# Raymond30/Krylov-Cubic-Regularized-Newton

Hardware: AMD Instinct MI355X
Metric: Hessian-vector products/sec + achieved HBM GB/s, news20 CSR, 1/2/4/8 MI355X (higher is better)
Workload: dtype f64; 1 GPU; news20: one device Lanczos (cubic.py:77-111) of m=100 HVPs per step; n=19996, d=1355191, nnz=9097916, m=100, partition=none, parallelism=single GPU

## Files before the change

krylov-cubic-regularized-newton_amd/csrc/krcn_geom.hpp:

```cpp
#pragma once
#include <stdint.h>

#include <cstdlib>
#include <cstring>

#include "krcn.h"

#ifdef __HIPCC__
#define KRCN_HD __host__ __device__
#else
#define KRCN_HD
#endif

namespace krcn {

constexpr int kNumCUs = 256;
constexpr int kNT = 256;
constexpr int kMaxPartials = 2048;

constexpr int kApplyU = 4;
inline int apply_grid(int64_t rows) {
  int64_t b = (rows + int64_t(kNT) * kApplyU - 1) / (int64_t(kNT) * kApplyU);
  return int(b < 1 ? 1 : (b > 1024 ? 1024 : b));
}

inline const char* tuning_env(const char* name) {
#ifdef KRCN_TUNING
  return getenv(name);
#else
  (void)name;
  return nullptr;
#endif
}
template <typename V>
inline V tuning_value(const char* name, V dflt, int field = 0) {
  const char* e = tuning_env(name);
  for (; e && field > 0; --field)
    if ((e = std::strchr(e, ',')) != nullptr) ++e;
  return e ? V(std::atof(e)) : dflt;
}
inline bool tuning_on(const char* name) {
  const char* e = tuning_env(name);
  return !(e && e[0] == '0');
}
inline bool tuning_off(const char* name) {
  const char* e = tuning_env(name);
  return e && e[0] == '1';
}

inline int auto_lanes(int64_t rows, int64_t nnz) {
  const double mean = rows > 0 ? double(nnz) / double(rows) : 0.0;
  int L = 1;
  while (L < 64 && double(L * 2) * 8.0 <= mean) L *= 2;
  return L;
}

inline int resolve_lanes(int policy, int64_t rows, int64_t nnz) {
  if (policy == KRCN_LANES_AUTO) return auto_lanes(rows, nnz);
  if (policy == KRCN_LANES_SEQUENTIAL) return 1;
  return policy;
}

struct __attribute__((aligned(32))) TileDesc {
  int slice, long_row, row0, row1, p0, p1, pad0, pad1;
};

constexpr int kWaveTileNnz = 512;
constexpr int kWaveTileRows = 128;
constexpr int kWavesPerBlock = kNT / 64;

constexpr int kCombineRows = 128;
constexpr int kCombineSpread = 256;
inline int combine_rows(int rows) {
  const int R = (rows + kCombineSpread - 1) / kCombineSpread;
  return R < 1 ? 1 : (R > kCombineRows ? kCombineRows : R);
}
inline int combine_grid(int rows) {
  const int R = combine_rows(rows);
  const int g = (rows + R - 1) / R;
  return g < 1 ? 1 : (g > kCombineSpread ? kCombineSpread : g);
}

constexpr int kSortPerThread = 8;
constexpr int ilog2(int v) { return v <= 1 ? 0 : 1 + ilog2(v / 2); }
template <int NT> struct SortGeom {
  static constexpr int kTile = NT * kSortPerThread;
  static constexpr int kRows = kTile / 4;
  static constexpr int kRowRegs = (kRows + 1 + NT - 1) / NT;
  static constexpr int kSlotBits = ilog2(kTile);
  static_assert((1 << kSlotBits) == kTile, "slot field must address a whole tile");
  static constexpr int64_t kMaxWindow = int64_t(1) << (32 - kSlotBits);
};

struct __attribute__((aligned(16))) WinSeg {
  int slice, t0, t1, flags;
};
enum { kSegLoad = 1, kSegFlush = 2 };

constexpr int kWinNT = 1024;
constexpr int kWinWaves = kWinNT / 64;
constexpr int kWinChunk = 256;
constexpr int kWinTMax = 6;
constexpr int kWinPad = kWinChunk + 8;
constexpr int kWinRing = 3;
constexpr int kWinBatch = 26;
template <typename T> struct WinGeom {
  static constexpr int kSlabBytes = kWinWaves * kWinChunk * int(sizeof(T));
  static constexpr int kBytes = 163840 - kSlabBytes - 256;
  static constexpr int kW = kBytes / int(sizeof(T));
  static constexpr int kPer = (kW + kWinNT - 1) / kWinNT;
  static_assert(kW <= 65536, "16-bit slice-local offsets");
};

KRCN_HD inline void win_block_slice(int b, int G, int S, int kpb, int& slice, int& chunk) {
  if (kpb == 0) {
    slice = b % S;
    chunk = b / S;
    return;
  }
  const int x = b % 8, q = G / 8, r = G % 8;
  const int slot = x * q + (x < r ? x : r) + b / 8;
  slice = slot / kpb;
  chunk = slot % kpb;
}

constexpr int kXtChunk = 4;
constexpr int kXtRowCap = kWinWaves * kWinTMax * 64;
constexpr unsigned short kXtPad = 0xFFFF;
template <typename T> struct XtGeom {
  static constexpr int kChunks = WinGeom<T>::kW - kWinNT - kXtRowCap;
};

constexpr int kJagNT = 1024;
constexpr int kJagWaves = kJagNT / 64;
constexpr int kJagLdsBytes = 163840 - 256;
constexpr int kJagPieces = kJagLdsBytes / 16;
constexpr int kJagSlab = 128;
constexpr int kJagPad = 2 * kJagSlab;

#ifndef KRCN_JAG_CPG
#define KRCN_JAG_CPG 2
#endif
constexpr int kJagK1 = 6, kJagCPG1 = KRCN_JAG_CPG, kJagLC = 8;
constexpr int kJagCPGU = 2;
constexpr int jag_cpg(int K) { return K <= 2 ? 2 : kJagCPG1; }
constexpr int kJagK2 = 8;
constexpr int kJagLong = 32, kJagTask = 128, kJagLongTasks = 256;

template <typename T> struct JagGeom {
  static constexpr int kE = 16 / int(sizeof(T));
  static constexpr int kW1 = kJagPieces * kE;
  static constexpr int kR1 = (kJagPieces + kJagNT - 1) / kJagNT;
  static constexpr int kPieces2 = (kJagLdsBytes - kJagWaves * (kJagSlab + 2) * int(sizeof(T))) / 32;
  static constexpr int kW2 = kPieces2 * kE;
  static constexpr int kR2 = (kPieces2 + kJagNT - 1) / kJagNT;
  static_assert(kW1 <= 65536, "16-bit slice-local offsets");
};

}
```

krylov-cubic-regularized-newton_amd/csrc/krcn_window.hpp:

```cpp
#pragma once
#include <type_traits>
#include <utility>

#include "krcn_tiled.hpp"

namespace krcn {

#ifndef KRCN_WIN_RING_ACCUM
#define KRCN_WIN_RING_ACCUM 2
#endif
constexpr int kWinRingAccum = KRCN_WIN_RING_ACCUM;
#ifndef KRCN_WIN_SUMU
#define KRCN_WIN_SUMU 8
#endif
#ifndef KRCN_WIN_COOP
#define KRCN_WIN_COOP 1
#endif
constexpr int kWinCoopLen = 64;
#ifndef KRCN_WIN_FIRST
#define KRCN_WIN_FIRST 1
#endif

struct WinArgs {
  int rows, W, stride, S;
  int dbg;
  int ntiles;
  int64_t cols;
  const int* tb;
  const unsigned short* ro;
  const unsigned short* widx;
  const void* wval;
  const WinSeg* segs;
  int kpb = 0;
};
template <bool kAccum>
__device__ __forceinline__ const int* win_tb(const WinArgs& a, int slice) {
  return a.tb + int64_t(slice) * ((kAccum ? 1 : 2) * (a.ntiles + 1));
}

typedef unsigned short u16x4 __attribute__((ext_vector_type(4)));

template <typename T> struct Quad;
template <> struct Quad<double> {
  __device__ __forceinline__ static void load(const double* p, double (&v)[4]) {
    const f64x2 a = *reinterpret_cast<const f64x2*>(p);
    const f64x2 b = *(reinterpret_cast<const f64x2*>(p) + 1);
    v[0] = a.x; v[1] = a.y; v[2] = b.x; v[3] = b.y;
  }
};
template <> struct Quad<float> {
  __device__ __forceinline__ static void load(const float* p, float (&v)[4]) {
    const f32x4 a = *reinterpret_cast<const f32x4*>(p);
    v[0] = a.x; v[1] = a.y; v[2] = a.z; v[3] = a.w;
  }
};

#ifdef KRCN_WIN_TIMING
constexpr int kWinDbgSlots = 32;
static __device__ unsigned long long krcn_win_dbg[3 * 2048 * kWinDbgSlots];
[[maybe_unused]] static int win_stamps_read(unsigned long long* out, int n, int reset) {
  if (hipDeviceSynchronize() != hipSuccess) return 1;
  if (hipMemcpyFromSymbol(out, HIP_SYMBOL(krcn_win_dbg), sizeof(unsigned long long) * n) != hipSuccess) return 1;
  if (reset) {
    static unsigned long long z[3 * 2048 * kWinDbgSlots];
    if (hipMemcpyToSymbol(HIP_SYMBOL(krcn_win_dbg), z, sizeof(z)) != hipSuccess) return 1;
  }
  return 0;
}
#define KRCN_WIN_STAMP(slot)                                                                          \
  do {                                                                                                \
    if (threadIdx.x == 0 && blockIdx.x < 2048)                                                        \
      krcn_win_dbg[a.dbg * 2048 * kWinDbgSlots + blockIdx.x * kWinDbgSlots + (slot)] =   \
          __builtin_amdgcn_s_memrealtime();                                                           \
  } while (0)
#define KRCN_WIN_WAVE_STAMP(slot)                                                                     \
  do {                                                                                                \
    if ((threadIdx.x & 63) == 0 && blockIdx.x < 2048)                                                 \
      krcn_win_dbg[a.dbg * 2048 * kWinDbgSlots + blockIdx.x * kWinDbgSlots + (slot)] =   \
          __builtin_amdgcn_s_memrealtime();                                                           \
  } while (0)
#else
#define KRCN_WIN_STAMP(slot) do {} while (0)
#define KRCN_WIN_WAVE_STAMP(slot) do {} while (0)
#endif

template <typename T, typename TS = T> struct WinChunk {
  u16x4 q;
  TS v[4];
  int c0, base, hi;
};

template <typename T, typename TS>
__device__ __forceinline__ void win_load(WinChunk<T, TS>& c, int c0, int e1, const unsigned short* __restrict__ widx,
                                         const TS* __restrict__ wval, int lane) {
  c.c0 = c0;
  c.base = c0 & ~3;
  c.hi = c.base + kWinChunk < e1 ? c.base + kWinChunk : e1;
  const int e = c.base + 4 * lane;
  c.q = *reinterpret_cast<const u16x4*>(widx + e);
  Quad<TS>::load(wval + e, c.v);
}

template <typename T, typename TS>
__device__ __forceinline__ T win_consume(const WinChunk<T, TS>& c, int beg, int end, const T* win, T* slab, int lane,
                                         T s, bool coop, T& open) {
  const int e = c.base + 4 * lane;
  const unsigned short qi[4] = {c.q.x, c.q.y, c.q.z, c.q.w};
#if defined(KRCN_WIN_ABL_NOSUM)
#pragma unroll
  for (int i = 0; i < 4; ++i) s += T(c.v[i]) * win[e + i < c.hi ? qi[i] : 0];
  (void)beg; (void)end; (void)slab; (void)coop; (void)open;
  return s;
#else
#pragma unroll
  for (int i = 0; i < 4; ++i) slab[4 * lane + i] = T(c.v[i]) * win[e + i < c.hi ? qi[i] : 0];
  wave_lds_sync();
  const int pb = beg > c.c0 ? beg : c.c0;
  const int pe = end < c.hi ? end : c.hi;
  int p = pb;
#if KRCN_WIN_SUMU > 1
  if (coop) {
    unsigned long long longm = __ballot(end - beg > kWinCoopLen && pe > pb);
    while (longm != 0ull) {
      const int L = __builtin_ctzll(longm);
      longm &= longm - 1ull;
      const int lb = __builtin_amdgcn_readlane(pb, L), le = __builtin_amdgcn_readlane(pe, L);
      const int rb = __builtin_amdgcn_readlane(beg, L), re = __builtin_amdgcn_readlane(end, L);
      T part = lb > rb ? open : T(0);
      for (int q = lb + ((lane - (lb - rb)) & 63); q < le; q += 64) part += slab[q - c.base];
      if (le < re) {
        open = part;
        continue;
      }
#pragma unroll
      for (int off = 32; off > 0; off >>= 1) part += __shfl_xor(part, off, 64);
      if (lane == L) s += part;
    }
    if (end - beg > kWinCoopLen) p = pe;
  }
  if (__ballot(pe - p > 2 * KRCN_WIN_SUMU) != 0ull) {
    for (; p + KRCN_WIN_SUMU <= pe; p += KRCN_WIN_SUMU) {
      T a[KRCN_WIN_SUMU];
#pragma unroll
      for (int u = 0; u < KRCN_WIN_SUMU; ++u) a[u] = slab[p + u - c.base];
#pragma unroll
      for (int u = 0; u < KRCN_WIN_SUMU; ++u) s += a[u];
    }
  }
#endif
  for (; p < pe; ++p) s += slab[p - c.base];
  wave_lds_sync();
  return s;
#endif
}

__device__ __forceinline__ void lds_block_barrier() {
  __builtin_amdgcn_fence(__ATOMIC_RELEASE, "workgroup", "local");
  __builtin_amdgcn_s_barrier();
  __builtin_amdgcn_fence(__ATOMIC_ACQUIRE, "workgroup", "local");
}

template <typename T>
__device__ __forceinline__ void win_fetch(T (&tmp)[WinGeom<T>::kPer], const T* __restrict__ x, int slice,
                                          const WinArgs& a, int rot) {
  constexpr int kPer = WinGeom<T>::kPer;
  const int64_t wbase = int64_t(slice) * a.W;
  const int len = a.cols - wbase < a.W ? int(a.cols - wbase) : a.W;
#pragma unroll
  for (int k = 0; k < kPer; ++k) {
    const int q = k + rot < kPer ? k + rot : k + rot - kPer;
    const int i = threadIdx.x + kWinNT * q;
    if (kWinNT * q < len) tmp[k] = x[wbase + (i < len ? i : len - 1)];
  }
}

template <typename T>
__device__ __forceinline__ void win_store(const T (&tmp)[WinGeom<T>::kPer], T* win, int slice, const WinArgs& a,
                                          int rot) {
  constexpr int kPer = WinGeom<T>::kPer;
  const int64_t wbase = int64_t(slice) * a.W;
  const int len = a.cols - wbase < a.W ? int(a.cols - wbase) : a.W;
#pragma unroll
  for (int k = 0; k < kPer; ++k) {
    const int q = k + rot < kPer ? k + rot : k + rot - kPer;
    const int i = threadIdx.x + kWinNT * q;
    if (i < len) win[i] = tmp[k];
  }
}

template <int... I, class F>
__device__ __forceinline__ void unroll_while(std::integer_sequence<int, I...>, int n, F&& f) {
  bool go = true;
  ((go = go && (I < n), go ? (f(std::integral_constant<int, I>{}), 0) : 0), ...);
}

template <int R>
struct TileB {
  int r0, nr, e0, e1;
  __device__ __forceinline__ void set(int rows, int t, int t1, int te0, int te1) {
    t = t < t1 ? t : t1 - 1;
    t = t > 0 ? t : 0;
    r0 = t * R;
    nr = rows - r0 < R ? rows - r0 : R;
    e0 = te0;
    e1 = te1;
  }
  __device__ __forceinline__ void set_rows(int tr0, int tr1, int te0, int te1) {
    r0 = tr0;
    nr = tr1 - tr0;
    e0 = te0;
    e1 = te1;
  }
};

struct WinTiles {
  int lo, hi, kb;
  template <bool kRows>
  __device__ __forceinline__ void load(const int* tb, int roff, int tw, int t1, int kb_, int lane) {
    kb = kb_;
    int t = tw + kWinWaves * (kb + (kRows ? lane & 31 : lane));
    t = t < t1 ? t : t1 - 1;
    t = t > 0 ? t : 0;
    if (kRows && lane >= 32) t += roff;
    lo = tb[t];
    hi = tb[t + 1];
  }
};

struct RowRaw {
  int o1, o0;
};
template <int R>
__device__ __forceinline__ RowRaw tile_row_load(const TileB<R>& b, const unsigned short* ro, int lane) {
  const int i1 = lane < b.nr ? lane : b.nr - 1;
  const int i0 = lane < b.nr ? (lane > 0 ? lane - 1 : 0) : b.nr - 1;
  return RowRaw{int(ro[b.r0 + i1]), int(ro[b.r0 + i0])};
}
template <int R>
__device__ __forceinline__ void tile_row_bounds(const TileB<R>& b, const RowRaw& q, int lane, int& bg, int& en) {
  const int ea = b.e0 + q.o1, eb = b.e0 + q.o0;
  en = lane < b.nr ? ea : b.e1;
  bg = lane < b.nr ? (lane > 0 ? eb : b.e0) : b.e1;
}

#ifndef KRCN_FOLD
#define KRCN_FOLD 0
#endif
#ifndef KRCN_FOLD_ABL
#define KRCN_FOLD_ABL 0
#endif
constexpr int kFoldPad = 32;
template <typename T> struct EpiSliceFold {
  T* part; int64_t ld;
  int* cnt;
  int* won;
  int* nwon;
  int ntiles;
  double* aq;
  const T* w; T* u;
  LzCtl<T> c;
  int S;
  static constexpr bool kReduce = false;
  struct Pre {};
  template <class Src> __device__ __forceinline__ void init(const Src&) {}
  __device__ __forceinline__ Pre pre(int) const { return Pre{}; }
  __device__ __forceinline__ double row(int r, T s, int slice, const Pre&) const {
    __hip_atomic_store(part + int64_t(slice) * ld + r, s, __ATOMIC_RELAXED, __HIP_MEMORY_SCOPE_AGENT);
    return 0.0;
  }
};
template <class E> struct IsFoldEpi : std::false_type {};
template <typename T> struct IsFoldEpi<EpiSliceFold<T>> : std::true_type {};

template <typename T>
__device__ __forceinline__ double fold_beta(const LzCtl<T>& c, int lane) {
  double g[kNT / 64];
#pragma unroll
  for (int w = 0; w < kNT / 64; ++w) {
    double v = 0.0;
    for (int i = 64 * w + lane; i < c.Pnorm; i += kNT) v += c.pnorm[i];
    g[w] = wave_sum(v);
  }
  return sqrt((g[0] + g[1]) + (g[2] + g[3]));
}

struct WinFold {
  int t1 = -1, t2 = -1;
  int a1 = -1, a2 = -1;
  int o1 = 0, o2 = 0;
  int bstate = 0;
  double beta = 0.0;
};

template <typename T, int R>
__device__ __forceinline__ void fold_combine(const EpiSliceFold<T>& e, WinFold& f, int t, int rows, int lane) {
  if constexpr (R != 32) {
    return;
  } else {
  if (f.bstate == 0) {
    const int done = e.c.j > 0 ? __hip_atomic_load(&e.c.st->done, __ATOMIC_RELAXED, __HIP_MEMORY_SCOPE_AGENT) : 0;
    f.beta = fold_beta(e.c, lane);
    f.bstate = (done || (e.c.j > 0 && fabs(f.beta) < e.c.tol)) ? 2 : 1;
  }
  const int r0 = t * R;
  if (f.bstate == 1) {
    __builtin_amdgcn_fence(__ATOMIC_ACQUIRE, "agent");
    const int p = lane & 15, q = lane >> 4;
    const int ra = r0 + 2 * p;
    const int rA = ra < rows ? ra : rows - 1, rB = ra + 1 < rows ? ra + 1 : rows - 1;
    T w0 = T(0), w1 = T(0);
    if (q == 0) {
      w0 = e.w[rA];
      w1 = e.w[rB];
    }
    constexpr int kH = 12;
    T v0a = T(0), v4a = T(0), v0b = T(0), v4b = T(0);
#pragma unroll
    for (int h = 0; h < 2; ++h) {
      T a0[kH], a1[kH];
#pragma unroll
      for (int k = 0; k < kH; ++k) {
        const int s = q + 4 * (h * kH + k);
        const T* pp = e.part + int64_t(s < e.S ? s : q) * e.ld;
        a0[k] = __hip_atomic_load(pp + rA, __ATOMIC_RELAXED, __HIP_MEMORY_SCOPE_AGENT);
        a1[k] = __hip_atomic_load(pp + rB, __ATOMIC_RELAXED, __HIP_MEMORY_SCOPE_AGENT);
      }
#pragma unroll
      for (int k = 0; k < kH; ++k)
        if (q + 4 * (h * kH + k) < e.S) {
          if (k % 2 == 0) { v0a += a0[k]; v0b += a1[k]; }
          else { v4a += a0[k]; v4b += a1[k]; }
        }
    }
    const T n0a = __shfl_down(v0a, 16, 64), n4a = __shfl_down(v4a, 16, 64);
    const T n0b = __shfl_down(v0b, 16, 64), n4b = __shfl_down(v4b, 16, 64);
    const T l1a = v0a + n0a, l5a = v4a + n4a, l1b = v0b + n0b, l5b = v4b + n4b;
    const T m1a = __shfl_down(l1a, 32, 64), m5a = __shfl_down(l5a, 32, 64);
    const T m1b = __shfl_down(l1b, 32, 64), m5b = __shfl_down(l5b, 32, 64);
    const T sa = (l1a + m1a) + (l5a + m5a), sb = (l1b + m1b) + (l5b + m5b);
    double acc = 0.0;
    if (q == 0) {
      const T div = T(f.beta);
      if (ra < rows) {
        const T qa = sa / div, ua = w0 * qa;
        e.u[ra] = ua;
        acc += double(ua) * double(qa);
      }
      if (ra + 1 < rows) {
        const T qb = sb / div, ub = w1 * qb;
        e.u[ra + 1] = ub;
        acc += double(ub) * double(qb);
      }
    }
    acc = wave_sum(acc);
    if (lane == 0) e.aq[t] = acc;
  } else if (lane == 0) {
    e.aq[t] = 0.0;
  }
  if (lane == 0) __hip_atomic_store(e.cnt + int64_t(t) * kFoldPad, 0, __ATOMIC_RELAXED, __HIP_MEMORY_SCOPE_AGENT);
  }
}

template <typename T>
__device__ __forceinline__ void fold_won(const EpiSliceFold<T>& e, int t, int lane) {
  if (lane == 0) {
    const int i = __hip_atomic_fetch_add(e.nwon, 1, __ATOMIC_RELAXED, __HIP_MEMORY_SCOPE_WORKGROUP);
    e.won[int64_t(blockIdx.x) * e.ntiles + i] = t;
  }
}

template <typename T, int R>
__device__ __forceinline__ void fold_after(const EpiSliceFold<T>& e, WinFold& f, int t, int rows, int lane) {
  if (f.a2 >= 0 && __builtin_amdgcn_readfirstlane(f.o2) == e.S - 1) fold_won(e, f.a2, lane);
  f.a2 = f.a1;
  f.o2 = f.o1;
  f.a1 = -1;
  if (f.t2 >= 0) {
    __builtin_amdgcn_s_waitcnt(0x0f78);
    int o = 0;
#if KRCN_FOLD_ABL
    if (lane == 0) o = f.t2 % 97 == 0 ? 0 : 1;
#else
    if (lane == 0) o = __hip_atomic_fetch_add(e.cnt + int64_t(f.t2) * kFoldPad, 1, __ATOMIC_RELAXED, __HIP_MEMORY_SCOPE_AGENT);
#endif
    f.o1 = o;
    f.a1 = f.t2;
  }
  f.t2 = f.t1;
  f.t1 = t;
}

template <typename T, int R>
__device__ __forceinline__ void fold_drain(const EpiSliceFold<T>& e, WinFold& f, int rows, int lane) {
  __builtin_amdgcn_s_waitcnt(0x0f70);
  int ta[4] = {f.a2, f.a1, f.t2, f.t1};
  int oa[4] = {f.o2, f.o1, 0, 0};
#pragma unroll
  for (int i = 2; i < 4; ++i)
    if (ta[i] >= 0) {
      int o = 0;
      if (lane == 0) o = __hip_atomic_fetch_add(e.cnt + int64_t(ta[i]) * kFoldPad, 1, __ATOMIC_RELAXED, __HIP_MEMORY_SCOPE_AGENT);
      oa[i] = o;
    }
#pragma unroll
  for (int i = 0; i < 4; ++i)
    if (ta[i] >= 0 && __builtin_amdgcn_readfirstlane(oa[i]) == e.S - 1) fold_won(e, ta[i], lane);
  f = WinFold{};
}

template <typename T, typename TS, int R, class Epi>
__device__ __forceinline__ void win_stream(int segno, const WinSeg& sg, const WinArgs& a,
                                           const T (&tmp)[WinGeom<T>::kPer], bool store_win, int rot, T* win,
                                           T* slab, const Epi& epi, int wave, int lane,
                                           typename RedOf<Epi>::type& red, WinTiles tl) {
  const int rows = a.rows;
  const int* tb = win_tb<false>(a, sg.slice);
  const unsigned short* ro = a.ro + int64_t(sg.slice) * rows;
  const unsigned short* widx = a.widx;
  const TS* wval = static_cast<const TS*>(a.wval);
  const int tw = sg.t0 + wave;
  const int nt = sg.t1 - tw > 0 ? (sg.t1 - tw + kWinWaves - 1) / kWinWaves : 0;
  const int nb = (nt + kWinBatch - 1) / kWinBatch;
  WinFold fold;
  if (nb == 0 && store_win) {
    lds_block_barrier();
    win_store<T>(tmp, win, sg.slice, a, rot);
    lds_block_barrier();
  }
  for (int bi = 0; bi < nb; ++bi) {
    const int kb = bi * kWinBatch;
    const int kn = nt - kb < kWinBatch ? nt - kb : kWinBatch;
    if (bi > 0) tl.load<true>(tb, a.ntiles + 1, tw, sg.t1, kb, lane);
    auto bounds = [&](TileB<R>& b, int k) {
      b.e0 = __builtin_amdgcn_readlane(tl.lo, k);
      b.e1 = __builtin_amdgcn_readlane(tl.hi, k);
    };
    TileB<R> B0, B1, B2;
    bounds(B0, 0);
    bounds(B1, 1);
    bounds(B2, 2);
    WinChunk<T, TS> c0, c1, c2;
    RowRaw q0, q1, q2;
    typename Epi::Pre p0, p1, p2;
    auto rows_of = [&](TileB<R>& b, int k, RowRaw& q, typename Epi::Pre& pr) {
      b.set_rows(__builtin_amdgcn_readlane(tl.lo, k + 32), __builtin_amdgcn_readlane(tl.hi, k + 32), b.e0, b.e1);
      q = tile_row_load<R>(b, ro, lane);
      const int r = b.r0 + lane;
      pr = epi.pre(r < rows ? r : rows - 1);
    };
    const bool sw = bi == 0 && store_win;
#if KRCN_WIN_FIRST
    if (sw) {
      lds_block_barrier();
      win_store<T>(tmp, win, sg.slice, a, rot);
    }
    rows_of(B0, 0, q0, p0);
    win_load(c0, B0.e0, B0.e1, widx, wval, lane);
    win_load(c1, B1.e0, B1.e1, widx, wval, lane);
    if (sw) lds_block_barrier();
#else
    rows_of(B0, 0, q0, p0);
    win_load(c0, B0.e0, B0.e1, widx, wval, lane);
    win_load(c1, B1.e0, B1.e1, widx, wval, lane);
    if (sw) {
      lds_block_barrier();
      win_store<T>(tmp, win, sg.slice, a, rot);
      lds_block_barrier();
    }
#endif
    if (segno < 4 && bi == 0) KRCN_WIN_STAMP(2 + 2 * segno);
    auto finish = [&](const WinChunk<T, TS>& c, const TileB<R>& b, const RowRaw& q, const typename Epi::Pre& pr,
                      int k) {
      int bg, en;
      tile_row_bounds<R>(b, q, lane, bg, en);
      const bool coop = KRCN_WIN_COOP && a.S > 1;
      T open = T(0);
      T s = win_consume(c, bg, en, win, slab, lane, T(0), coop, open);
      for (int cc = c.hi; cc < b.e1;) {
        WinChunk<T, TS> cx;
        win_load(cx, cc, b.e1, widx, wval, lane);
        s = win_consume(cx, bg, en, win, slab, lane, s, coop, open);
        cc = cx.hi;
      }
      if (k < kn && lane < b.nr) red += epi.row(b.r0 + lane, s, sg.slice, pr);
      if constexpr (IsFoldEpi<Epi>::value)
        if (k < kn) fold_after<T, R>(epi, fold, b.r0 / R, rows, lane);
    };
    for (int k = 0; k < kn; k += 3) {
      rows_of(B1, k + 1, q1, p1);
      win_load(c2, B2.e0, B2.e1, widx, wval, lane);
      finish(c0, B0, q0, p0, k);
      bounds(B0, k + 3);
      rows_of(B2, k + 2, q2, p2);
      win_load(c0, B0.e0, B0.e1, widx, wval, lane);
      finish(c1, B1, q1, p1, k + 1);
      bounds(B1, k + 4);
      rows_of(B0, k + 3, q0, p0);
      win_load(c1, B1.e0, B1.e1, widx, wval, lane);
      finish(c2, B2, q2, p2, k + 2);
      bounds(B2, k + 5);
    }
  }
  if constexpr (IsFoldEpi<Epi>::value) fold_drain<T, R>(epi, fold, rows, lane);
}

template <typename T, typename TS, int R, class Epi, bool FLUSH>
__device__ __forceinline__ void win_accum(int segno, const WinSeg& sg, const WinArgs& a, const T (&tmp)[WinGeom<T>::kPer],
                                          bool store_win, int rot, T* win, T* slab, const Epi& epi, int wave,
                                          int lane, T (&acc)[kWinTMax], typename RedOf<Epi>::type& red,
                                          const WinTiles& tl) {
  constexpr int K = kWinTMax;
  constexpr int D = kWinRingAccum;
  const int rows = a.rows;
  const unsigned short* ro = a.ro + int64_t(sg.slice) * rows;
  const unsigned short* widx = a.widx;
  const TS* wval = static_cast<const TS*>(a.wval);
  const int nt = sg.t1 - sg.t0 - wave > 0 ? (sg.t1 - sg.t0 - wave + kWinWaves - 1) / kWinWaves : 0;
  TileB<R> B[K];
#pragma unroll
  for (int k = 0; k < K; ++k)
    B[k].set(rows, sg.t0 + wave + k * kWinWaves, sg.t1, __builtin_amdgcn_readlane(tl.lo, k),
             __builtin_amdgcn_readlane(tl.hi, k));
  WinChunk<T, TS> ring[D];
  RowRaw rq[D];
  typename Epi::Pre pre[D];
  auto issue_chunk = [&](auto kc) {
    constexpr int k = decltype(kc)::value;
    win_load(ring[k % D], B[k].e0, B[k].e1, widx, wval, lane);
  };
  auto issue_rows = [&](auto kc) {
    constexpr int k = decltype(kc)::value;
    rq[k % D] = tile_row_load<R>(B[k], ro, lane);
    if constexpr (FLUSH) {
      const int r = B[k].r0 + lane;
      pre[k % D] = epi.pre(r < rows ? r : rows - 1);
    }
  };
#if KRCN_WIN_FIRST
  if (store_win) {
    lds_block_barrier();
    win_store<T>(tmp, win, sg.slice, a, rot);
  }
  issue_rows(std::integral_constant<int, 0>{});
  issue_chunk(std::integral_constant<int, 0>{});
  if constexpr (K > 1 && D > 2) issue_chunk(std::integral_constant<int, 1>{});
  if (store_win) lds_block_barrier();
#else
  issue_rows(std::integral_constant<int, 0>{});
  issue_chunk(std::integral_constant<int, 0>{});
  if constexpr (K > 1 && D > 2) issue_chunk(std::integral_constant<int, 1>{});
  if (store_win) {
    lds_block_barrier();
    win_store<T>(tmp, win, sg.slice, a, rot);
    lds_block_barrier();
  }
#endif
  if (segno < 4) KRCN_WIN_STAMP(2 + 2 * segno);
  auto step = [&](auto kc) {
    constexpr int k = decltype(kc)::value;
    if constexpr (k + 1 < K) issue_rows(std::integral_constant<int, k + 1>{});
    if constexpr (k + D - 1 < K && D > 1) issue_chunk(std::integral_constant<int, k + D - 1>{});
    const WinChunk<T, TS>& cur = ring[k % D];
    int bg, en;
    tile_row_bounds<R>(B[k], rq[k % D], lane, bg, en);
    T none = T(0);
    T s = win_consume(cur, bg, en, win, slab, lane, acc[k], false, none);
    for (int c = cur.hi; c < B[k].e1;) {
      WinChunk<T, TS> cx;
      win_load(cx, c, B[k].e1, widx, wval, lane);
      s = win_consume(cx, bg, en, win, slab, lane, s, false, none);
      c = cx.hi;
    }
    if constexpr (FLUSH) {
      if (lane < B[k].nr) red += epi.row(B[k].r0 + lane, s, sg.slice, pre[k % D]);
      acc[k] = T(0);
    } else {
      acc[k] = s;
    }
  };
  unroll_while(std::make_integer_sequence<int, K>{}, nt, step);
}

template <typename T> struct EpiLz1X {
  const T* w; T div;
  const int* xcp;
  const unsigned short* xrow;
  const T* xval;
  T* part;
  int cols;
  T* lu; int rbase;
  static constexpr bool kReduce = false;
  static constexpr bool kPreEarly = true;
  struct Pre { T wr; };
  template <class S> __device__ __forceinline__ void init(const S& src) { div = src.v.div; }
  __device__ __forceinline__ Pre pre(int r) const { return Pre{w[r]}; }
  __device__ __forceinline__ double row(int r, T s, int, const Pre& p) const {
    lu[r - rbase] = p.wr * (s / div);
    return 0.0;
  }
  __device__ __forceinline__ void xt(int b, T* tp) const {
    const int* cp = xcp + int64_t(b) * (cols + 1);
    const int c = threadIdx.x;
    const int cb = cp[0], ce = cp[cols];
    int c0 = 0, c1 = 0;
    if (c < cols) {
      c0 = cp[c];
      c1 = cp[c + 1];
    }
    for (int t = cb + int(threadIdx.x); t < ce; t += kWinNT) {
      T v[kXtChunk];
      Quad<T>::load(xval + int64_t(t) * kXtChunk, v);
      const u16x4 q = *reinterpret_cast<const u16x4*>(xrow + int64_t(t) * kXtChunk);
      const unsigned short rr[kXtChunk] = {q.x, q.y, q.z, q.w};
      T s = T(0);
#pragma unroll
      for (int i = 0; i < kXtChunk; ++i) {
        const T pr = v[i] * lu[rr[i] != kXtPad ? rr[i] : 0];
        if (rr[i] != kXtPad) s += pr;
      }
      tp[t - cb] = s;
    }
    __builtin_amdgcn_fence(__ATOMIC_RELEASE, "workgroup", "local");
    __builtin_amdgcn_s_barrier();
    __builtin_amdgcn_fence(__ATOMIC_ACQUIRE, "workgroup", "local");
    if (c < cols) {
      T s = T(0);
      for (int k = c0; k < c1; ++k) s += tp[k - cb];
      part[int64_t(b) * cols + c] = s;
    }
  }
};
template <class E> struct IsEpiXt : std::false_type {};
template <typename T> struct IsEpiXt<EpiLz1X<T>> : std::true_type {};


template <typename T, typename TS, int R, class Src, class Epi, bool kAccum>
__global__ __launch_bounds__(kWinNT, 1) void k_window_pass(WinArgs a, Src src, Epi epi,
                                                           double* __restrict__ partials) {
  constexpr int kPer = WinGeom<T>::kPer;
  __shared__ double sm[kWinNT / 64];
  __shared__ T win[WinGeom<T>::kW];
  __shared__ T slab_all[kWinWaves][kWinChunk];
  __shared__ int fold_n;
  if constexpr (IsFoldEpi<Epi>::value) {
    if (threadIdx.x == 0) fold_n = 0;
    epi.nwon = &fold_n;
  }
  KRCN_WIN_STAMP(0);
  const WinSeg* bsegs = a.segs + int64_t(blockIdx.x) * a.stride;
  WinSeg sg = bsegs[0];
  const int nseg = sg.flags >> 8;
  const int rot = int((blockIdx.x >> 3) % kPer);
  int slice0 = sg.slice, chunk0 = 0;
  if constexpr (!kAccum) win_block_slice(int(blockIdx.x), int(gridDim.x), a.S, a.kpb, slice0, chunk0);
  WinTiles tl;
  if constexpr (kAccum)
    tl.template load<false>(win_tb<true>(a, sg.slice), 0, sg.t0 + __builtin_amdgcn_readfirstlane(int(threadIdx.x) >> 6),
                            sg.t1, 0, int(threadIdx.x) & 63);
  T tmp[kPer];
  const T* x = nullptr;
  if constexpr (IsLzZ<Src>::value) {
    const int j = src.c.j;
    T tv[kPer];
    const bool early = src.Pa <= kNT;
    int flag = 0;
    double pv = 0.0;
    if (j > 0 && early) {
      if (threadIdx.x == 0) flag = __hip_atomic_load(&src.c.st->done, __ATOMIC_RELAXED, __HIP_MEMORY_SCOPE_AGENT);
      if (threadIdx.x < src.Pa) pv = src.pa[threadIdx.x];
    }
    win_fetch<T>(tmp, j == 0 ? src.c.g : src.Wv, slice0, a, rot);
    if (j > 0) win_fetch<T>(tv, src.c.V + int64_t(j - 1) * src.c.ld, slice0, a, rot);
    if (j > 0 && early) {
      __shared__ int flag_sm;
      if (threadIdx.x == 0) flag_sm = flag;
      __syncthreads();
      const int done = flag_sm;
      __syncthreads();
      if (done) return;
      const double al = block_sum(threadIdx.x < kNT ? 0.0 + pv : 0.0, sm);
      if (blockIdx.x == 0 && threadIdx.x == 0) src.alphas[j - 1] = al;
      src.alpha = T(al);
    } else if (src.begin(sm)) {
      return;
    }
    if (j > 0) {
      const int64_t wbase = int64_t(slice0) * a.W;
      const int len = a.cols - wbase < a.W ? int(a.cols - wbase) : a.W;
      const T ta = src.alpha;
#pragma unroll
      for (int k = 0; k < kPer; ++k) tmp[k] = tmp[k] - ta * tv[k];
      const int kpb = a.kpb ? a.kpb : int(gridDim.x) / a.S, cb = chunk0;
      T* z = src.c.V + int64_t(j) * src.c.ld + wbase;
      double nrm = 0.0;
#pragma unroll
      for (int k = 0; k < kPer; ++k) {
        const int q = k + rot < kPer ? k + rot : k + rot - kPer;
        const int i = threadIdx.x + kWinNT * q;
        if (q % kpb == cb && i < len) {
          if (src.store_z) store_policy<KRCN_VEC_ST>(z + i, tmp[k]);
          nrm += double(tmp[k]) * double(tmp[k]);
        }
      }
      const double bs = block_sum_nt<kWinNT>(nrm, sm);
      if (threadIdx.x == 0) src.pz[blockIdx.x] = bs;
    }
  } else if constexpr (IsLzSmall<Src>::value) {
    const int j = src.c.j;
    const int t = threadIdx.x;
    const int64_t d = src.c.ld;
    const bool in = t < d;
    const int tc = in ? t : 0;
    const T wv = (j == 0 ? src.c.g : src.Wv)[tc];
    const T vv = j == 0 ? T(0) : (src.c.V + int64_t(j - 1) * d)[tc];
    double al = 0.0;
    if (j > 0 && flag_and_sum(&src.c.st->done, src.pa, src.Pa, sm, &al)) return;
    const T zi = j == 0 ? wv : wv - T(al) * vv;
    const double nrm = sqrt(block_sum_nt<kWinNT>(in ? double(zi) * double(zi) : 0.0, sm));
    const bool lead = blockIdx.x == 0 && t == 0;
    if (j == 0) {
      if (lead) { src.c.st->done = 0; src.c.st->j_break = -1; src.c.st->gnorm = nrm; src.c.st->beta_last = 0.0; }
    } else {
      if (lead) src.alphas[j - 1] = al;
      if (fabs(nrm) < src.c.tol) {
        if (lead) { src.c.st->j_break = j - 1; src.c.st->beta_last = nrm; src.c.st->done = 1; }
        return;
      }
      if (lead) { src.c.betas[j - 1] = nrm; src.c.st->beta_last = nrm; }
      if (blockIdx.x == 0 && in) src.c.V[int64_t(j) * d + t] = zi;
    }
    src.v = LzVec<T>{j == 0 ? src.c.g : src.c.V + int64_t(j) * d, T(nrm), j, 1};
#pragma unroll
    for (int k = 0; k < kPer; ++k) tmp[k] = (k + rot) % kPer == 0 ? zi : T(0);
  } else {
    if constexpr (HasPreload<Src>::value) src.preload();
    const T* xe = src.early();
    win_fetch<T>(tmp, xe, slice0, a, rot);
    if (src.begin(sm)) return;
    x = src.get();
    if (x != xe) win_fetch<T>(tmp, x, slice0, a, rot);
  }
  KRCN_WIN_STAMP(1);
  if constexpr (!kAccum)
    tl.template load<true>(win_tb<false>(a, sg.slice), a.ntiles + 1,
                           sg.t0 + __builtin_amdgcn_readfirstlane(int(threadIdx.x) >> 6), sg.t1, 0,
                           int(threadIdx.x) & 63);
  epi.init(src);
  if constexpr (IsEpiXt<Epi>::value) {
    epi.lu = win + kWinNT;
    epi.rbase = sg.t0 * R;
  }
  const int wave = __builtin_amdgcn_readfirstlane(threadIdx.x >> 6), lane = threadIdx.x & 63;
  T* slab = slab_all[wave];
  typename RedOf<Epi>::type red{};
  T acc[kWinTMax];
#pragma unroll
  for (int k = 0; k < kWinTMax; ++k) acc[k] = T(0);
  for (int si = 0; si < nseg; ++si) {
    bool store_win = si == 0;
    if (si > 0) {
      sg = bsegs[si];
      tl.template load<!kAccum>(win_tb<kAccum>(a, sg.slice), a.ntiles + 1, sg.t0 + wave, sg.t1, 0, lane);
      if (sg.flags & kSegLoad) {
        win_fetch<T>(tmp, x, sg.slice, a, rot);
        store_win = true;
      }
    }
    if constexpr (kAccum) {
      if (sg.flags & kSegFlush)
        win_accum<T, TS, R, Epi, true>(si, sg, a, tmp, store_win, rot, win, slab, epi, wave, lane, acc, red, tl);
      else
        win_accum<T, TS, R, Epi, false>(si, sg, a, tmp, store_win, rot, win, slab, epi, wave, lane, acc, red, tl);
    } else {
      win_stream<T, TS, R, Epi>(si, sg, a, tmp, store_win, rot, win, slab, epi, wave, lane, red, tl);
    }
    if (si < 4) KRCN_WIN_STAMP(3 + 2 * si);
  }
  KRCN_WIN_WAVE_STAMP(16 + wave);
  if constexpr (IsEpiXt<Epi>::value) {
    lds_block_barrier();
    epi.xt(int(blockIdx.x), win + kWinNT + kXtRowCap);
  }
  if constexpr (IsFoldEpi<Epi>::value) {
    __syncthreads();
    const int nw = fold_n;
    WinFold f;
    for (int i = wave; i < nw; i += kWinWaves)
      fold_combine<T, R>(epi, f, epi.won[int64_t(blockIdx.x) * epi.ntiles + i], a.rows, lane);
  }
  if constexpr (Epi::kReduce) store_block_red<kWinNT>(red, sm, partials, epi);
  KRCN_WIN_STAMP(10);
}

[[maybe_unused]] static __global__ __launch_bounds__(kNT) void k_compact_rows(int S, int rows, int R, int ntiles,
                                                      const int* __restrict__ ptr, int* __restrict__ tb,
                                                      unsigned short* __restrict__ ro) {
  const int64_t total = int64_t(S) * rows;
  for (int64_t i = int64_t(blockIdx.x) * kNT + threadIdx.x; i < total; i += int64_t(gridDim.x) * kNT) {
    const int sl = int(i / rows), r = int(i % rows);
    const int t = r / R;
    const int base = ptr[int64_t(sl) * rows + int64_t(t) * R];
    ro[i] = static_cast<unsigned short>(ptr[i + 1] - base);
    if (r % R == 0) tb[int64_t(sl) * (ntiles + 1) + t] = base;
    if (r == rows - 1) tb[int64_t(sl) * (ntiles + 1) + ntiles] = ptr[int64_t(sl) * rows + rows];
  }
}

[[maybe_unused]] static __global__ __launch_bounds__(kNT) void k_compact_tiles(int S, int rows, int ntiles,
                                                       const int* __restrict__ ptr, const int* __restrict__ tb,
                                                       unsigned short* __restrict__ ro) {
  const int64_t total = int64_t(S) * ntiles;
  for (int64_t i = int64_t(blockIdx.x) * kNT + threadIdx.x; i < total; i += int64_t(gridDim.x) * kNT) {
    const int sl = int(i / ntiles), t = int(i % ntiles);
    const int* rp = ptr + int64_t(sl) * rows;
    const int* q = tb + int64_t(sl) * 2 * (ntiles + 1);
    const int base = q[t], r0 = q[ntiles + 1 + t], r1 = q[ntiles + 2 + t];
    for (int r = r0; r < r1; ++r) ro[int64_t(sl) * rows + r] = static_cast<unsigned short>(rp[r + 1] - base);
  }
}

[[maybe_unused]] static __global__ __launch_bounds__(kNT) void k_local_u16(int64_t nnz, const int* __restrict__ idx, int W,
                                                   unsigned short* __restrict__ out) {
  for (int64_t e = int64_t(blockIdx.x) * kNT + threadIdx.x; e < nnz; e += int64_t(gridDim.x) * kNT)
    out[e] = static_cast<unsigned short>(idx[e] % W);
}

}
```

Baseline: 17820 HVP/s.

## Replace static per-wave tile striding with LDS atomic dynamic tile claiming in window stream

The streaming window pass used to give each wave a fixed stride of tiles, preloaded in batches. Now each wave keeps its first three static tiles, then claims the rest one at a time from a shared LDS counter with atomics. This evens out load across waves when tile costs differ, which matters for skewed CSR rows. The cost is an atomic plus a tile-bound global load per tile, extra barriers to reset the counter for each segment, and the fold epilogue path being statically disallowed.

```diff
diff --git a/krylov-cubic-regularized-newton_amd/csrc/krcn_geom.hpp b/krylov-cubic-regularized-newton_amd/csrc/krcn_geom.hpp
--- a/krylov-cubic-regularized-newton_amd/csrc/krcn_geom.hpp
+++ b/krylov-cubic-regularized-newton_amd/csrc/krcn_geom.hpp
@@ -103,7 +103,10 @@
 constexpr int kWinTMax = 6;
 constexpr int kWinPad = kWinChunk + 8;
 constexpr int kWinRing = 3;
-constexpr int kWinBatch = 26;
+#ifndef KRCN_WIN_CLAIM
+#define KRCN_WIN_CLAIM 1
+#endif
+constexpr int kWinClaimRun = KRCN_WIN_CLAIM;
 template <typename T> struct WinGeom {
   static constexpr int kSlabBytes = kWinWaves * kWinChunk * int(sizeof(T));
   static constexpr int kBytes = 163840 - kSlabBytes - 256;
@@ -122,6 +125,30 @@
   const int slot = x * q + (x < r ? x : r) + b / 8;
   slice = slot / kpb;
   chunk = slot % kpb;
+}
+
+KRCN_HD inline int win_claim_start(int t0, int t1) {
+  const int n = t1 - t0, p = kWinWaves * kWinRing;
+  return t0 + (n < p ? (n > 0 ? n : 0) : p);
+}
+KRCN_HD inline int win_static_tile(int t0, int t1, int w, int k) {
+  const int t = t0 + w + kWinWaves * k;
+  return t < t1 ? t : -1;
+}
+struct WinRun {
+  int first, n;
+};
+KRCN_HD inline WinRun win_claim_run(int t0, int t1, int c, int run = kWinClaimRun) {
+  const int start = win_claim_start(t0, t1);
+  const int pool = t1 > start ? t1 - start : 0;
+  const int before = c <= pool / run ? c * run : pool;
+  const int taken = before < pool ? before : pool;
+  const int left = pool - taken;
+  return WinRun{start + taken, left < run ? left : run};
+}
+KRCN_HD inline int win_tile_clamp(int t, int t1) {
+  t = t < t1 ? t : t1 - 1;
+  return t > 0 ? t : 0;
 }
 
 constexpr int kXtChunk = 4;
diff --git a/krylov-cubic-regularized-newton_amd/csrc/krcn_window.hpp b/krylov-cubic-regularized-newton_amd/csrc/krcn_window.hpp
--- a/krylov-cubic-regularized-newton_amd/csrc/krcn_window.hpp
+++ b/krylov-cubic-regularized-newton_amd/csrc/krcn_window.hpp
@@ -412,96 +412,129 @@
 __device__ __forceinline__ void win_stream(int segno, const WinSeg& sg, const WinArgs& a,
                                            const T (&tmp)[WinGeom<T>::kPer], bool store_win, int rot, T* win,
                                            T* slab, const Epi& epi, int wave, int lane,
-                                           typename RedOf<Epi>::type& red, WinTiles tl) {
+                                           typename RedOf<Epi>::type& red, const WinTiles& tl, int* claim) {
+  static_assert(!IsFoldEpi<Epi>::value,
+                "KRCN_FOLD indexes a wave's tiles statically: not ported to the claimed tiles of win_stream");
+  static_assert(kWinClaimRun >= 1 && kWinRing == 3, "the ring below is written out for three slots");
   const int rows = a.rows;
   const int* tb = win_tb<false>(a, sg.slice);
+  const int roff = a.ntiles + 1;
   const unsigned short* ro = a.ro + int64_t(sg.slice) * rows;
   const unsigned short* widx = a.widx;
   const TS* wval = static_cast<const TS*>(a.wval);
-  const int tw = sg.t0 + wave;
-  const int nt = sg.t1 - tw > 0 ? (sg.t1 - tw + kWinWaves - 1) / kWinWaves : 0;
-  const int nb = (nt + kWinBatch - 1) / kWinBatch;
-  WinFold fold;
-  if (nb == 0 && store_win) {
+  if (win_static_tile(sg.t0, sg.t1, wave, 0) < 0) {
+    if (store_win) {
+      lds_block_barrier();
+      win_store<T>(tmp, win, sg.slice, a, rot);
+      lds_block_barrier();
+    }
+    return;
+  }
+  struct Tile {
+    TileB<R> b;
+    bool ok;
+  };
+  auto from_prefix = [&](Tile& x, int k) {
+    x.ok = win_static_tile(sg.t0, sg.t1, wave, k) >= 0;
+    const int e0 = __builtin_amdgcn_readlane(tl.lo, k);
+    const int e1 = __builtin_amdgcn_readlane(tl.hi, k);
+    x.b.set_rows(__builtin_amdgcn_readlane(tl.lo, k + 32), __builtin_amdgcn_readlane(tl.hi, k + 32), e0, x.ok ? e1 : e0);
+  };
+  Tile X0, X1, X2;
+  from_prefix(X0, 0);
+  from_prefix(X1, 1);
+  from_prefix(X2, 2);
+  int clv = 0;
+  int cbv = 0;
+  bool okn = false;
+  WinRun rn{0, 0};
+  int sub = kWinClaimRun;
+  int* const claim_at = lane == 0 ? claim : reinterpret_cast<int*>(slab) + lane;
+  auto claim_issue = [&]() {
+    clv = __hip_atomic_fetch_add(claim_at, lane == 0 ? 1 : 0, __ATOMIC_RELAXED, __HIP_MEMORY_SCOPE_WORKGROUP);
+  };
+  auto fetch_next = [&]() {
+    if (kWinClaimRun == 1 || sub == kWinClaimRun) {
+      rn = win_claim_run(sg.t0, sg.t1, __builtin_amdgcn_readfirstlane(clv));
+      claim_issue();
+      sub = 0;
+    }
+    okn = sub < rn.n;
+    const int t = win_tile_clamp(rn.first + sub, sg.t1);
+    ++sub;
+    cbv = tb[t + (lane & 1) + ((lane & 2) ? roff : 0)];
+  };
+  auto take = [&](Tile& x) {
+    x.ok = okn;
+    const int e0 = __builtin_amdgcn_readlane(cbv, 0);
+    const int e1 = __builtin_amdgcn_readlane(cbv, 1);
+    x.b.set_rows(__builtin_amdgcn_readlane(cbv, 2), __builtin_amdgcn_readlane(cbv, 3), e0, okn ? e1 : e0);
+  };
+  WinChunk<T, TS> c0, c1, c2;
+  RowRaw q0, q1, q2;
+  typename Epi::Pre p0, p1, p2;
+  auto rows_of = [&](const Tile& x, RowRaw& q, typename Epi::Pre& pr) {
+    q = tile_row_load<R>(x.b, ro, lane);
+    const int r = x.b.r0 + lane;
+    pr = epi.pre(r < rows ? r : rows - 1);
+  };
+#if KRCN_WIN_FIRST
+  if (store_win) {
+    lds_block_barrier();
+    win_store<T>(tmp, win, sg.slice, a, rot);
+  }
+  rows_of(X0, q0, p0);
+  win_load(c0, X0.b.e0, X0.b.e1, widx, wval, lane);
+  win_load(c1, X1.b.e0, X1.b.e1, widx, wval, lane);
+  claim_issue();
+  if (store_win) lds_block_barrier();
+#else
+  rows_of(X0, q0, p0);
+  win_load(c0, X0.b.e0, X0.b.e1, widx, wval, lane);
+  win_load(c1, X1.b.e0, X1.b.e1, widx, wval, lane);
+  if (store_win) {
     lds_block_barrier();
     win_store<T>(tmp, win, sg.slice, a, rot);
     lds_block_barrier();
   }
-  for (int bi = 0; bi < nb; ++bi) {
-    const int kb = bi * kWinBatch;
-    const int kn = nt - kb < kWinBatch ? nt - kb : kWinBatch;
-    if (bi > 0) tl.load<true>(tb, a.ntiles + 1, tw, sg.t1, kb, lane);
-    auto bounds = [&](TileB<R>& b, int k) {
-      b.e0 = __builtin_amdgcn_readlane(tl.lo, k);
-      b.e1 = __builtin_amdgcn_readlane(tl.hi, k);
-    };
-    TileB<R> B0, B1, B2;
-    bounds(B0, 0);
-    bounds(B1, 1);
-    bounds(B2, 2);
-    WinChunk<T, TS> c0, c1, c2;
-    RowRaw q0, q1, q2;
-    typename Epi::Pre p0, p1, p2;
-    auto rows_of = [&](TileB<R>& b, int k, RowRaw& q, typename Epi::Pre& pr) {
-      b.set_rows(__builtin_amdgcn_readlane(tl.lo, k + 32), __builtin_amdgcn_readlane(tl.hi, k + 32), b.e0, b.e1);
-      q = tile_row_load<R>(b, ro, lane);
-      const int r = b.r0 + lane;
-      pr = epi.pre(r < rows ? r : rows - 1);
-    };
-    const bool sw = bi == 0 && store_win;
-#if KRCN_WIN_FIRST
-    if (sw) {
-      lds_block_barrier();
-      win_store<T>(tmp, win, sg.slice, a, rot);
-    }
-    rows_of(B0, 0, q0, p0);
-    win_load(c0, B0.e0, B0.e1, widx, wval, lane);
-    win_load(c1, B1.e0, B1.e1, widx, wval, lane);
-    if (sw) lds_block_barrier();
-#else
-    rows_of(B0, 0, q0, p0);
-    win_load(c0, B0.e0, B0.e1, widx, wval, lane);
-    win_load(c1, B1.e0, B1.e1, widx, wval, lane);
-    if (sw) {
-      lds_block_barrier();
-      win_store<T>(tmp, win, sg.slice, a, rot);
-      lds_block_barrier();
-    }
-#endif
-    if (segno < 4 && bi == 0) KRCN_WIN_STAMP(2 + 2 * segno);
-    auto finish = [&](const WinChunk<T, TS>& c, const TileB<R>& b, const RowRaw& q, const typename Epi::Pre& pr,
-                      int k) {
-      int bg, en;
-      tile_row_bounds<R>(b, q, lane, bg, en);
-      const bool coop = KRCN_WIN_COOP && a.S > 1;
-      T open = T(0);
-      T s = win_consume(c, bg, en, win, slab, lane, T(0), coop, open);
-      for (int cc = c.hi; cc < b.e1;) {
-        WinChunk<T, TS> cx;
-        win_load(cx, cc, b.e1, widx, wval, lane);
-        s = win_consume(cx, bg, en, win, slab, lane, s, coop, open);
-        cc = cx.hi;
-      }
-      if (k < kn && lane < b.nr) red += epi.row(b.r0 + lane, s, sg.slice, pr);
-      if constexpr (IsFoldEpi<Epi>::value)
-        if (k < kn) fold_after<T, R>(epi, fold, b.r0 / R, rows, lane);
-    };
-    for (int k = 0; k < kn; k += 3) {
-      rows_of(B1, k + 1, q1, p1);
-      win_load(c2, B2.e0, B2.e1, widx, wval, lane);
-      finish(c0, B0, q0, p0, k);
-      bounds(B0, k + 3);
-      rows_of(B2, k + 2, q2, p2);
-      win_load(c0, B0.e0, B0.e1, widx, wval, lane);
-      finish(c1, B1, q1, p1, k + 1);
-      bounds(B1, k + 4);
-      rows_of(B0, k + 3, q0, p0);
-      win_load(c1, B1.e0, B1.e1, widx, wval, lane);
-      finish(c2, B2, q2, p2, k + 2);
-      bounds(B2, k + 5);
-    }
-  }
-  if constexpr (IsFoldEpi<Epi>::value) fold_drain<T, R>(epi, fold, rows, lane);
+  claim_issue();
+#endif
+  if (segno < 4) KRCN_WIN_STAMP(2 + 2 * segno);
+  auto finish = [&](const WinChunk<T, TS>& c, const Tile& x, const RowRaw& q, const typename Epi::Pre& pr) {
+    const TileB<R>& b = x.b;
+    int bg, en;
+    tile_row_bounds<R>(b, q, lane, bg, en);
+    const bool coop = KRCN_WIN_COOP && a.S > 1;
+    T open = T(0);
+    T s = win_consume(c, bg, en, win, slab, lane, T(0), coop, open);
+    for (int cc = c.hi; cc < b.e1;) {
+      WinChunk<T, TS> cx;
+      win_load(cx, cc, b.e1, widx, wval, lane);
+      s = win_consume(cx, bg, en, win, slab, lane, s, coop, open);
+      cc = cx.hi;
+    }
+    if (x.ok && lane < b.nr) red += epi.row(b.r0 + lane, s, sg.slice, pr);
+  };
+  for (;;) {
+    fetch_next();
+    rows_of(X1, q1, p1);
+    win_load(c2, X2.b.e0, X2.b.e1, widx, wval, lane);
+    finish(c0, X0, q0, p0);
+    take(X0);
+    if (!X1.ok) break;
+    fetch_next();
+    rows_of(X2, q2, p2);
+    win_load(c0, X0.b.e0, X0.b.e1, widx, wval, lane);
+    finish(c1, X1, q1, p1);
+    take(X1);
+    if (!X2.ok) break;
+    fetch_next();
+    rows_of(X0, q0, p0);
+    win_load(c1, X1.b.e0, X1.b.e1, widx, wval, lane);
+    finish(c2, X2, q2, p2);
+    take(X2);
+    if (!X0.ok) break;
+  }
 }
 
 template <typename T, typename TS, int R, class Epi, bool FLUSH>
@@ -642,6 +675,7 @@
   __shared__ T win[WinGeom<T>::kW];
   __shared__ T slab_all[kWinWaves][kWinChunk];
   __shared__ int fold_n;
+  __shared__ int claim;
   if constexpr (IsFoldEpi<Epi>::value) {
     if (threadIdx.x == 0) fold_n = 0;
     epi.nwon = &fold_n;
@@ -650,6 +684,8 @@
   const WinSeg* bsegs = a.segs + int64_t(blockIdx.x) * a.stride;
   WinSeg sg = bsegs[0];
   const int nseg = sg.flags >> 8;
+  if constexpr (!kAccum)
+    if (threadIdx.x == 0) claim = 0;
   const int rot = int((blockIdx.x >> 3) % kPer);
   int slice0 = sg.slice, chunk0 = 0;
   if constexpr (!kAccum) win_block_slice(int(blockIdx.x), int(gridDim.x), a.S, a.kpb, slice0, chunk0);
@@ -765,6 +801,11 @@
         win_fetch<T>(tmp, x, sg.slice, a, rot);
         store_win = true;
       }
+      if constexpr (!kAccum) {
+        lds_block_barrier();
+        if (threadIdx.x == 0) claim = 0;
+        if (!store_win) lds_block_barrier();
+      }
     }
     if constexpr (kAccum) {
       if (sg.flags & kSegFlush)
@@ -772,7 +813,7 @@
       else
         win_accum<T, TS, R, Epi, false>(si, sg, a, tmp, store_win, rot, win, slab, epi, wave, lane, acc, red, tl);
     } else {
-      win_stream<T, TS, R, Epi>(si, sg, a, tmp, store_win, rot, win, slab, epi, wave, lane, red, tl);
+      win_stream<T, TS, R, Epi>(si, sg, a, tmp, store_win, rot, win, slab, epi, wave, lane, red, tl, &claim);
     }
     if (si < 4) KRCN_WIN_STAMP(3 + 2 * si);
   }
```

Result: faster. 18250 HVP/s, median of 6 (+2.4%).
